# Simencassiman/P2PMicrogrid

Measured on AMD Instinct MI355X. Metric: agent-steps/sec (whole node, rollout+Q-update) at 1/2/4/8 MI355X; % HBM roofline, higher is better.
Workload: dtype f32 simulation, f64 Q-table

## Files before the change

p2pmicrogrid_amd/csrc/p2pmg_fast.hip:

```cpp
#include "p2pmg_fastmath.h"

namespace p2pmg {
namespace {

template <typename QT>
__device__ __forceinline__ Row4<QT> fake_row(const QT* p) {
  const uint32_t x = (uint32_t)(reinterpret_cast<uintptr_t>(p) >> 5);
  return Row4<QT>{{(QT)(x & 3), (QT)((x >> 2) & 3), (QT)((x >> 4) & 3), (QT)0}};
}

template <int N, int D, int G>
__device__ __forceinline__ void gather_even(float ev, float (&col)[N], int i) {
  if constexpr (D < G) {
    const float got = shfl_xor_c<D>(ev);
    const int src = i ^ D;
#pragma unroll
    for (int k = 0; k < N; ++k) col[k] = (k == src) ? got : col[k];
    gather_even<N, D + 1, G>(ev, col, i);
  }
}

#ifndef P2PMG_BAT_SPEC
#define P2PMG_BAT_SPEC 1
#endif
// ... 53 lines not shown
    bk = BatK{p.bat_min, p.bat_max, p.bat_sqrt_eff, recip64_u(p.bat_sqrt_eff), kR900};
    rcap = recip64(bcap > 0.0 ? bcap : 1.0);
  }
  const int ip_zero = idx_plain(div_n<N>(0.0f) / mi, np);
  QT* const q_dummy = reinterpret_cast<QT*>(p.dummy) + lane * kQPad;
  constexpr bool narrow = NARROW;
  const size_t rec_bytes = narrow ? sizeof(float2) : sizeof(FastRec);
  char* const rec_dummy = reinterpret_cast<char*>(reinterpret_cast<FastRec*>(p.dummy) + kWave + lane);
  const bool rec_on = p.record != 0 && active;
  const size_t rec_step = rec_on ? A * rec_bytes : 0;

  auto temp_bin = [&](float t_in) {
    const float x = t_in - k.setpoint;
    return clamp_bin_f(((x + 1.0f) / 2.0f) * km2_T + 1.0f, km1_T);
  };
  auto p2p_bin = [&](float x) { return clamp_bin_f(((x + 1.0f) / 2.0f) * kp, km1_p); };

  const float* envb = p.env + (size_t)s_env * kEnvStride;
  const size_t env_step = (size_t)p.n_env * kEnvStride;
  const uint2* preb = pre + a;
  const uint32_t* ipc_a = p.pre_ipc + a;
  const int t1 = T > 1 ? 1 : 0, t2 = 2 % T;
  const int n_chain = p.chain > 1 ? p.chain : 1;
  bool st_on = active;
  size_t rec_adv = rec_step;
  bool wrap_l = false;
  bool wrap_it = false;
  QT* snap = nullptr;
  if constexpr (PIPE) {
    __shared__ QT snap_lds[2 * 32 * 32];
    snap = snap_lds;
  }
  const uint32_t* codes_a;
  char* rec_ptr;
  uint32_t TA, env_st, env_end, o3, eo3;
  EnvV eS[3];
  uint2 pS[3];
  uint32_t cS[3];
  uint32_t cw, strip, a0, aN;
  int iT;
  Row4<QT> row0, rowN;
  uint32_t iS[3] = {0u, 0u, 0u};
  Row4<QT> cand[3];
  Patch<QT> pat{0xFFFFFFFFu, 0, (QT)0};
  float ep_sum = 0.0f;
  float t0_in = tin, t0_m = tm;
  auto code_of = [&](uint32_t w) { return TRAIN ? w : 0xFFFFFFFFu; };
  auto strip_of = [&](uint32_t base, int it_) { return __umul24(base + __umul24((uint32_t)it_, (uint32_t)nbv), (uint32_t)np); };
  auto row0_addr = [&](uint32_t st, uint32_t nr, uint32_t c) -> uint32_t {
    const bool need = ((c & 0xFF) == 255) || (TRAIN && R1 == 1);
    return need ? st + (uint32_t)ip_zero : nr;
  };
#if P2PMG_TRACE
  uint64_t trW = 0, trC = 0, trR = 0, trLast = 0, trA0 = 0, trWC = 0, trA1 = 0, trMid = 0, trCal = 0;
#define P2PMG_STAMP(v) asm volatile("s_memtime %0\n s_waitcnt lgkmcnt(0)" : "=s"(v)::"memory")
#endif
  auto begin_episode = [&](int ep) __attribute__((always_inline)) {
    if constexpr (PIPE) {
      if (ep >= 1 && st_on) {
        tin = t0_in;
        tm = t0_m;
      }
    }
    codes_a = p.codes + (size_t)(PIPE && ep < 0 ? 0 : ep) * p.codes_stride + a;
    if constexpr (PIPE) {
      rec_ptr = rec_on && st_on ? reinterpret_cast<char*>(recs) + (size_t)a * rec_bytes : rec_dummy;
      rec_adv = st_on ? rec_step : 0;
    } else {
      rec_ptr = rec_on ? reinterpret_cast<char*>(recs) + (size_t)a * rec_bytes : rec_dummy;
    }
    TA = (uint32_t)T * (uint32_t)A, env_st = (uint32_t)env_step, env_end = env_st * (uint32_t)T;
    o3 = (uint32_t)(3 % T) * (uint32_t)A, eo3 = (uint32_t)(3 % T) * env_st;

    eS[0] = load_envv(envb), eS[1] = load_envv(envb + (size_t)t1 * env_step), eS[2] = load_envv(envb + (size_t)t2 * env_step);
    pS[0] = preb[0], pS[1] = preb[(size_t)t1 * A], pS[2] = preb[(size_t)t2 * A];
    cS[0] = codes_a[0], cS[1] = codes_a[(size_t)t1 * A], cS[2] = codes_a[(size_t)t2 * A];
    cw = code_of(cS[0]);
    iT = temp_bin(tin);
    strip = strip_of(pS[0].y & 0xFFFFu, iT);
    const uint32_t nrow = strip_of(pS[0].y >> 16, iT) + (uint32_t)ip_zero;
    a0 = row0_addr(strip, nrow, cw);
    aN = TRAIN ? nrow : a0;
    row0 = gat(a0);
    rowN = gat(aN);
    if constexpr (CAND) {
      iS[0] = ipc_a[0];
      iS[1] = ipc_a[(size_t)t1 * A];
      iS[2] = ipc_a[(size_t)t2 * A];
#pragma unroll
      for (int b = 0; b < 3; ++b) cand[b] = gat((strip + ((iS[0] >> (8 * b)) & 0xFFu)));
    }
    pat = Patch<QT>{0xFFFFFFFFu, 0, (QT)0};
    ep_sum = 0.0f;
    if constexpr (!PIPE) {
      t0_in = tin, t0_m = tm;
      if (p.reset_t0 && active)
        t0_draw(p.seed_lo, p.seed_hi, p.episode + ep + 1, p.agent_offset + (uint32_t)a, k.setpoint, p.reset_sigma, t0_in,
                t0_m);
    } else {
      constexpr int kSnap = 10;
      const uint32_t key0 = pS[0].y & 0xFFFFu;
      const int nTi = p.nT;
      Row4<QT> sr[kSnap];
      auto snap_load = [&](int it0) {
#pragma unroll
        for (int j = 0; j < kSnap; ++j) sr[j] = gat(strip_of(key0, it0 + j < nTi ? it0 + j : nTi - 1) + (uint32_t)ip_zero);
      };
      auto snap_store = [&](int it0) {
#pragma unroll
        for (int j = 0; j < kSnap; ++j)
          if (it0 + j < nTi) snap[(grp * 32 + it0 + j) * 32 + hl] = max3(sr[j]);
      };
      snap_load(0);
      if (active)
        t0_draw(p.seed_lo, p.seed_hi, p.episode + (ep + 2 < n_chain ? ep + 2 : n_chain), p.agent_offset + (uint32_t)a,
                k.setpoint, p.reset_sigma, t0_in, t0_m);
      snap_store(0);
      for (int it0 = kSnap; it0 < nTi; it0 += kSnap) {
        snap_load(it0);
        snap_store(it0);
      }
    }
  };
  auto end_episode = [&](int ep) __attribute__((always_inline)) {
    if (active) {
      if (p.reset_t0) {
        tin = t0_in;
        tm = t0_m;
      }
      if (i == 0) {
        if (p.chain_rewards) p.chain_rewards[(size_t)ep * p.S + s] = ep_sum;
        if (ep == n_chain - 1) p.ep_reward[s] = ep_sum;
      }
    }
  };

  auto step = [&](auto par) __attribute__((always_inline)) {
    constexpr int P = decltype(par)::value, P1 = (P + 1) % 3;
    const EnvV ev = eS[P];
    const EnvRow e0{0.0f, ev.x, ev.y, ev.z, ev.w};
    const uint2 p0 = pS[P], p1 = pS[P1];
    const uint32_t c1 = cS[P1], ipc0 = iS[P], ipc1 = iS[P1];
    const float balw = __uint_as_float(p0.x);
    float row[N];
    float col[N];
#pragma unroll
    for (int j = 0; j < N; ++j) { row[j] = 0.0f; col[j] = 0.0f; }
    float tinA[3];
    uint32_t iTA[3], stA[3], nrA[3];
    {
      const float ain = k.inv_ri * (tm - tin) + k.inv_rvent * (e0.t_out - tin);
#pragma unroll
      for (int x = 0; x < 3; ++x) {
// ... 38 lines not shown
    float tin1 = tin, tm1 = tm;
    int iT1 = 0;
    uint32_t strip1 = 0, cw1 = 0, a0n = 0, aNn = 0;
    Row4<QT> row0n, rowNn, candn[3];
    Sel3M mnext{};
    auto issue_next = [&](int act_final) {
      const Sel3M m = sel3_masks(act_final);
      mnext = m;
      strip1 = __float_as_uint(sel3(m, __uint_as_float(stA[0]), __uint_as_float(stA[1]), __uint_as_float(stA[2])));
      const uint32_t nrow1 =
          __float_as_uint(sel3(m, __uint_as_float(nrA[0]), __uint_as_float(nrA[1]), __uint_as_float(nrA[2])));
      cw1 = code_of(c1);
      a0n = row0_addr(strip1, nrow1, cw1);
      aNn = TRAIN ? nrow1 : a0n;
#if P2PMG_ABLATE == 8 || P2PMG_ABLATE == 10
      row0n = fake_row(q + a0n * kQPad);
      rowNn = fake_row(q + aNn * kQPad);
#else
      {
        Row4<QT> r0{};
        if (((cw1 & 0xFF) == 255) || (TRAIN && R1 == 1)) r0 = gat(a0n);
        row0n = r0;
      }
#endif
      if constexpr (CAND) {
#pragma unroll
        for (int b = 0; b < 3; ++b) candn[b] = gat((strip1 + ((ipc1 >> (8 * b)) & 0xFFu)));
      }
#if !(P2PMG_ABLATE == 8 || P2PMG_ABLATE == 10)
      rowNn = gat(aNn);
#endif
    };
    auto refill_words = [&]() {
      cS[P] = codes_a[o3];
      if constexpr (CAND) iS[P] = ipc_a[o3];
    };
    auto settle_next = [&]() {
      const Sel3M& m = mnext;
      iT1 = (int)__float_as_uint(sel3(m, __uint_as_float(iTA[0]), __uint_as_float(iTA[1]), __uint_as_float(iTA[2])));
      tin1 = sel3(m, tinA[0], tinA[1], tinA[2]);
      const float d_m = k.inv_cm * (((k.inv_ri * (tin - tm) + k.inv_re * (e0.t_out - tm)) + k.solar) +
                                    sel3(m, hm[0], hm[1], hm[2]));
      tm1 = tm + (d_m * k.spm) * k.slot;
    };
    if constexpr (R1 == 1) {
      issue_next(act);
      refill_words();
      settle_next();
    }
    float out0 = balw + hp;
    if constexpr (BAT != 0) {
      if (bcap > 0.0) out0 = bat_rule(out0, soc_r);
    }
    const float ev0 = div_n_r<N>(out0 * 1.0f, rn);
#pragma unroll
    for (int j = 0; j < N; ++j) row[j] = ev0;
#pragma unroll
    for (int r = 1; r < R1; ++r) {
      if (r == 1) {
        gather_even<N, 1, G>(ev0, col, i);
      } else {
        exchange<N>(row, col, i, sl, nullptr);
      }
      code = (int)((cw >> (8 * r)) & 0xFF);
      if (CAND && r == 1) {
        const int b = __float_as_int(shfl_xor_c<1>(__int_as_float(act)));
#if P2PMG_TRACE
// ... 159 lines not shown
      rp[0] = make_float4(rw, cost, g, pp);
      rp[1] = make_float4(tin, __uint_as_float(acts), __uint_as_float(bins), __uint_as_float(ips));
    }
    rec_ptr += PIPE ? rec_adv : rec_step;
    asm volatile("" ::: "memory");
    eS[P] = load_envv(envb + eo3);
    pS[P] = preb[o3];
    const float m = group_sum<N>(rw, lane, i, sl, nullptr);
    ep_sum = ep_sum + div_n_r<N>(m, rn);

    tin = tin1;
    tm = tm1;
    iT = iT1;
    o3 += (uint32_t)A;
    o3 = o3 == TA ? 0u : o3;
    eo3 += env_st;
    eo3 = eo3 == env_end ? 0u : eo3;
    strip = strip1;
    cw = cw1;
    a0 = a0n;
    aN = aNn;
    row0 = row0n;
    rowN = rowNn;
    if constexpr (CAND) {
#pragma unroll
      for (int b = 0; b < 3; ++b) cand[b] = candn[b];
    }
  };
  using S0 = std::integral_constant<int, 0>;
  using S1 = std::integral_constant<int, 1>;
  using S2 = std::integral_constant<int, 2>;
  if constexpr (!PIPE) {
    for (int ep = 0; ep < n_chain; ++ep) {
      begin_episode(ep);
      __builtin_amdgcn_s_waitcnt(0);
      int t = 0;
      for (; t + 3 <= T; t += 3) {
        step(S0{});
        step(S1{});
        step(S2{});
      }
      if (t < T) step(S0{});
      if (t + 1 < T) step(S1{});
#if P2PMG_TRACE
      if (threadIdx.x == 0 && (blockIdx.x == 0 || (int)blockIdx.x == n_cons / 2 || (int)blockIdx.x == n_cons - 1))
        printf("TRACE blk %d/%d T %d: per step wait %.1f round0 %.1f waitcand %.1f round1 %.1f issue %.1f rest %.1f "
               "(one stamp %.1f)\n",
               (int)blockIdx.x, n_cons, T, (double)trW / T, (double)trA0 / T, (double)trWC / T, (double)trA1 / T,
               (double)trC / T, (double)trR / (T - 1), (double)trCal / T);
      trW = trC = trR = trLast = trA0 = trWC = trA1 = trMid = trCal = 0;
#endif
      end_episode(ep);
    }
    if (active) {
      p.t_in[a] = tin;
      p.t_m[a] = tm;
      if constexpr (BAT != 0) p.soc[a] = soc;
    }
  } else {
    const int L = T / 2;
    int ep_l = grp == 0 ? 0 : -1;
    st_on = active && grp == 0;
    begin_episode(ep_l);
    __builtin_amdgcn_s_waitcnt(0);
    for (int ph = 0;; ++ph) {
      if (ph > 0) {
        if (grp == (ph & 1)) {
          if (st_on && i == 0) {
            if (p.chain_rewards) p.chain_rewards[(size_t)ep_l * p.S + s] = ep_sum;
            if (ep_l == n_chain - 1) p.ep_reward[s] = ep_sum;
          }
          if (ph <= n_chain) {
            ep_l = ph;
            st_on = active && ph < n_chain;
            begin_episode(ph < n_chain ? ph : n_chain - 1);
          }
        }
        __builtin_amdgcn_s_waitcnt(0);
        if (ph > n_chain) break;
      }
      wrap_l = st_on && grp != (ph & 1) && ep_l + 1 < n_chain;
      for (int t = 0; t < L; t += 3) {
        wrap_it = t + 3 >= L;
        step(S0{});
        step(S1{});
        step(S2{});
      }
    }
    if (active && grp == ((n_chain - 1) & 1)) {
      p.t_in[a] = t0_in;
      p.t_m[a] = t0_m;
    }
  }
}

template <int N>
constexpr bool kFastPipe = N == 2;

template <int N, typename QT, int R1, int BAT, bool NARROW>
void launch_fast_nw(const EpisodeParams& p, const uint2* pre, FastRec* recs, int blocks, int spw, int prod,
                    const PrepOut& nxt, hipEvent_t ev0, hipEvent_t ev1, hipStream_t st) {
  if constexpr (kFastPipe<N> && BAT == 0) {
    if (p.mode == 0 && p.interleave)
      return hipExtLaunchKernelGGL((episode_fast_kernel<N, QT, R1, true, BAT, NARROW, true>), dim3(blocks + prod),
                                   dim3(kWave), 0, st, ev0, ev1, 0, p, pre, recs, spw, blocks, nxt);
  }
  if (p.mode == 0)
    hipExtLaunchKernelGGL((episode_fast_kernel<N, QT, R1, true, BAT, NARROW>), dim3(blocks + prod), dim3(kWave), 0, st,
                          ev0, ev1, 0, p, pre, recs, spw, blocks, nxt);
  else
    hipExtLaunchKernelGGL((episode_fast_kernel<N, QT, R1, false, BAT, NARROW>), dim3(blocks + prod), dim3(kWave), 0, st,
                          ev0, ev1, 0, p, pre, recs, spw, blocks, nxt);
}
template <int N, typename QT, int R1, int BAT>
void launch_fast_b(const EpisodeParams& p, const uint2* pre, FastRec* recs, int blocks, int spw, int prod,
                   const PrepOut& nxt, hipEvent_t ev0, hipEvent_t ev1, hipStream_t st) {
  if (p.rec_narrow) return launch_fast_nw<N, QT, R1, BAT, true>(p, pre, recs, blocks, spw, prod, nxt, ev0, ev1, st);
  launch_fast_nw<N, QT, R1, BAT, false>(p, pre, recs, blocks, spw, prod, nxt, ev0, ev1, st);
}
template <int N, typename QT, int R1>
void launch_fast_r(const EpisodeParams& p, const uint2* pre, FastRec* recs, int blocks, int spw, int prod,
// ... 73 lines not shown
```

p2pmicrogrid_amd/csrc/p2pmg_fastmath.h:

```cpp
#pragma once
#include "p2pmg_tabular.h"

namespace p2pmg {
namespace {

struct Recip {
  float b, y;
  bool ok;
};
__device__ __forceinline__ bool in_div_range(float x) {
  const float m = fabsf(x);
  return m >= 0x1p-40f && m <= 0x1p40f;
}
__device__ __forceinline__ Recip recip(float b) {
  const float y0 = __builtin_amdgcn_rcpf(b);
  return Recip{b, __builtin_fmaf(__builtin_fmaf(-b, y0, 1.0f), y0, y0), in_div_range(b)};
}
__device__ __forceinline__ float fdiv_core(float a, const Recip& d) {
  const float q0 = a * d.y;
  const float r = __builtin_fmaf(-d.b, q0, a);
  const float q = __builtin_fmaf(r, d.y, q0);
  return __builtin_copysignf(q, q0);
}
__device__ __forceinline__ bool fdiv_ok(float a) {
// ... 26 lines not shown
  const double ang = 6.283185307179586 * u2;
  t_in = (float)((double)setpoint + sigma * (rad * cos(ang)));
  t_m = (float)((double)setpoint + sigma * (rad * sin(ang)));
}
__device__ __forceinline__ void prepass_one(const EpisodeParams& p, const PrepOut& o, size_t k, int ep = 0) {
  const int t = (int)(k / p.A), a = (int)(k % p.A);
  const int tn = t + 1 == p.T ? 0 : t + 1;
  const int se = p.n_env == 1 ? 0 : a / p.N;
  const float mi = p.max_in[a];
  const float2 f = p.prof[k], fn = p.prof[(size_t)tn * p.A + a];
  const float bal = (f.x - f.y) / mi, baln = (fn.x - fn.y) / mi;
  const float time_t = p.env[((size_t)t * p.n_env + se) * kEnvStride];
  const float time_n = p.env[((size_t)tn * p.n_env + se) * kEnvStride];
  const uint32_t tb = (uint32_t)(p.nT * p.nb);
  const uint32_t lo = (uint32_t)idx_time(time_t, p.nt) * tb + (uint32_t)idx_plain(bal, p.nb);
  const uint32_t hi = (uint32_t)idx_time(time_n, p.nt) * tb + (uint32_t)idx_plain(baln, p.nb);
  if (ep == 0) o.pre[k] = make_uint2(__float_as_uint(bal * mi), lo | (hi << 16));
  if (o.ipc && ep == 0) {
    const int i = a % 2, ap = a ^ 1;
    const float2 fp = p.prof[(size_t)t * p.A + ap];
    const float mip = p.max_in[ap];
    const float balw_p = ((fp.x - fp.y) / mip) * mip;
    const float4 lvp = p.hp_lv[ap];
    const float hpl[3] = {lvp.x, lvp.y, lvp.z};
    uint32_t ipc = 0;
    for (int b = 0; b < 3; ++b) {
      const float ev = div_n<2>((balw_p + hpl[b]) * 1.0f);
      float acc = 0.0f;
      for (int j = 0; j < 2; ++j) acc = acc + (-((j == i) ? 0.0f : ev));
      ipc |= (uint32_t)idx_plain(div_n<2>(acc) / mi, p.np) << (8 * b);
    }
    o.ipc[k] = ipc;
  }
  if (o.words) {
    EpisodeParams q = p;
    const bool chain = o.n_ep > 1;
    q.episode = o.episode + ep;
    q.eps = o.eps;
    q.eps_thr = chain ? o.ep_thr[ep] : o.eps_thr;
    q.eps_all = chain ? (int)((o.ep_all >> ep) & 1u) : o.eps_all;
    const int R1 = p.R + 1, W = (R1 + 3) >> 2;
    const uint32_t gid = p.agent_offset + (uint32_t)a;
    const uint64_t codes = philox_codes_of(q, t, gid);
    uint32_t* words = o.words + (size_t)ep * o.words_stride;
    for (int w = 0; w < W; ++w)
      words[((size_t)t * W + w) * p.A + a] =
          w < 2 ? (uint32_t)(codes >> (32 * w))
                : philox_code_word(t, R1, w, (uint32_t)q.episode, gid, q.eps_thr, q.eps_all, p.seed_lo, p.seed_hi);
  }
}

struct Recip64 {
  double d, y;
  bool ok;
};
__device__ __forceinline__ bool in_div_range64(double x) {
  const double m = fabs(x);
  return m >= 0x1p-300 && m <= 0x1p300;
}
__device__ __forceinline__ Recip64 recip64(double d) {
  const double r0 = __builtin_amdgcn_rcp(d);
  const double r1 = __builtin_fma(r0, __builtin_fma(-d, r0, 1.0), r0);
  return Recip64{d, __builtin_fma(r1, __builtin_fma(-d, r1, 1.0), r1), in_div_range64(d)};
}
constexpr Recip64 kR900{900.0, 1.0 / 900.0, true};
__device__ __forceinline__ double fdiv64_ieee(double n, double d) {
// ... 111 lines not shown
```

p2pmicrogrid_amd/csrc/p2pmg_internal.h:

```cpp
#pragma once
#include <hip/hip_runtime.h>
#include <stdint.h>

namespace p2pmg {

constexpr int kEnvStride = 8;
constexpr int kQPad = 4;
constexpr int kWave = 64;
constexpr int kMaxAgents = 64;
constexpr int kMaxRounds1 = 4096;
inline constexpr int general_tile_cap(int n) { return n <= 16 ? 16 : (n <= 32 ? 32 : 64); }
constexpr double kDeltaScale = 1099511627776.0;
constexpr int kDeltaCopies = 8;

struct EpisodeParams {
  int S, N, R, T, A;
  int mode, rng, episode, record;
  int n_env;
  const float* env;
  const float2* prof;
  const uint2* sqp;
  const float* max_in;
  float* t_in;
  float* t_m;
  void* q;
  const uint32_t* codes;
  double eps;
  uint32_t eps_thr;
  int eps_all;
  uint32_t seed_lo, seed_hi;
  uint32_t agent_offset;
  float* rec_reward;
  float* rec_cost;
  float* rec_grid;
  float* rec_p2p;
  float* rec_tin;
  uint8_t* rec_action;
  int32_t* rec_index;
  float* ep_reward;
  int shared_q;
  long long* qdelta;
  int battery;
  double* soc;
  const double* bat_cap;
  double bat_min, bat_max, bat_sqrt_eff;
  int bat_safe;
  const float4* hp_lv;
  const float4* thermal;
  void* dummy;
  uint32_t* pre_ipc;
  void* rec_pack;
  int rec_narrow;
  int reset_t0;
  double reset_sigma;
  int chain;
  int interleave;
  size_t codes_stride;
  float* chain_rewards;
  int nt, nT, nb, np;
  double alpha, gamma;
  float hp_levels[4];
  float setpoint, margin, lower, upper;
  float inv_ci, inv_cm, inv_ri, inv_re, inv_rvent, c_in, c_m, solar, cop, spm, slot;
  float mph, kilo, penw;
};

constexpr int kNetStride = 4672;
constexpr int kOffW1 = 0, kOffB1 = 320, kOffW2 = 384, kOffB2 = 4480, kOffW3 = 4544, kOffB3 = 4608;
constexpr int kDqnParams = 4609;
constexpr int kDqnBatch = 32;
constexpr int kTrans = 10;
constexpr uint32_t kTagSample = 0x5EED0100u;

struct DqnParams {
  EpisodeParams e;
  int t;
  int n_nets;
  float* theta;
  float* target;
  float* adam_m;
  float* adam_v;
  float* grad;
  float* segs;
  int seg_first;
  int n_segs;
  int seg_agents;
  int bps;
// ... 18 lines not shown
  int adam_pending;
  int adam_tpb;
  int fold_spt;
};
hipError_t launch_dqn_act(const DqnParams& p, hipStream_t stream);
hipError_t launch_dqn_sample(const DqnParams& p, hipStream_t stream);
hipError_t launch_dqn_sample_prepass(const DqnParams& p, uint16_t* out, hipStream_t stream);
hipError_t launch_dqn_train(const DqnParams& p, int blocks, bool shared_partials, hipStream_t stream);
int dqn_train_blocks_per_cu();
hipError_t launch_dqn_reduce_adam(const DqnParams& p, int segments, bool adam, hipStream_t stream);
hipError_t launch_dqn_adam_shared(const DqnParams& p, hipStream_t stream);
constexpr int kActAdamSegs = 8;
bool dqn_act_fuses_adam(const DqnParams& p);
hipError_t launch_dqn_forward(const float* theta, int n, const float* x, float* q, hipStream_t stream);

struct RcParams {
  float inv_ci, inv_cm, inv_ri, inv_re, inv_rvent, c_in, c_m, solar, cop, spm, slot;
};

hipError_t launch_episode(const EpisodeParams& p, int q_dtype, int tile, hipStream_t stream);
constexpr int kMaxChain = 64;
struct PrepOut {
  uint2* pre;
  uint32_t* ipc;
  uint32_t* words;
  int episode;
  double eps;
  uint32_t eps_thr;
  int eps_all;
  int n_ep;
  size_t words_stride;
  uint32_t ep_thr[kMaxChain];
  uint64_t ep_all;
};
inline void eps_threshold(double eps, uint32_t& thr, int& all) {
  double c = __builtin_ceil(eps * 4294967296.0);
  if (!(c > 0.0)) c = 0.0;
  all = c >= 4294967296.0 ? 1 : 0;
  thr = all ? 0xFFFFFFFFu : (uint32_t)c;
}
hipError_t launch_step_prepass(const EpisodeParams& p, const PrepOut& o, hipStream_t stream);
constexpr int kChainLagMaxT = 512;
hipError_t launch_chain_lag(int T, int A, const uint2* pre, int* out, hipStream_t stream);
hipError_t launch_episode_fast(const EpisodeParams& p, const uint2* pre, void* recs, int q_dtype, int spw,
                               const PrepOut* next, hipEvent_t ev0, hipEvent_t ev1, hipStream_t stream);
#define P2PMG_DECL_FAST(name)                                                                                     \
  hipError_t name(const EpisodeParams& p, const uint2* pre, void* recs, int q_dtype, int spw, const PrepOut* next, \
                  hipEvent_t ev0, hipEvent_t ev1, hipStream_t stream);
P2PMG_DECL_FAST(launch_fast_n12)
P2PMG_DECL_FAST(launch_fast_n34)
P2PMG_DECL_FAST(launch_fast_n56)
P2PMG_DECL_FAST(launch_fast_n78)
hipError_t launch_general_n1_4(const EpisodeParams& p, int q_dtype, hipStream_t stream);
hipError_t launch_general_n5_8(const EpisodeParams& p, int q_dtype, hipStream_t stream);
hipError_t launch_general_n16(const EpisodeParams& p, int q_dtype, hipStream_t stream);
hipError_t launch_general_tile16(const EpisodeParams& p, int q_dtype, int nc, hipStream_t stream);
hipError_t launch_general_tile32_64(const EpisodeParams& p, int q_dtype, int nc, hipStream_t stream);
hipError_t launch_role_n1_4(const EpisodeParams& p, int q_dtype, hipStream_t stream);
hipError_t launch_role_n5_8(const EpisodeParams& p, int q_dtype, hipStream_t stream);
hipError_t launch_role_n16_tile16(const EpisodeParams& p, int q_dtype, int nc, hipStream_t stream);
hipError_t launch_role_tile32_64(const EpisodeParams& p, int q_dtype, int nc, hipStream_t stream);
hipError_t launch_rule_episode(const EpisodeParams& p, float* hp_on, hipStream_t stream);
hipError_t launch_episode_sq16(const EpisodeParams& p, int q_dtype, hipEvent_t ev0, hipEvent_t ev1, hipStream_t stream);
hipError_t launch_sq16_prep(const EpisodeParams& p, uint2* out, hipStream_t stream);
constexpr size_t kFastRecBytes = 32;
constexpr int kFastBatMaxR1 = 2;
// ... 65 lines not shown
```

p2pmicrogrid_amd/csrc/p2pmg_runtime.cpp:

```cpp
#include "p2pmg.h"

#include <dlfcn.h>
#include <hip/hip_runtime.h>

#include <algorithm>
#include <climits>
#include <cmath>
#include <cstdint>
#include <cstdio>
#include <cstdlib>
#include <cstring>
#include <new>
#include <string>
#include <vector>

#include "p2pmg_internal.h"
#include "p2pmg_plan.h"

using p2pmg::EpisodeParams;
using p2pmg::EpisodePlan;
using p2pmg::Family;
using p2pmg::kEnvStride;
using p2pmg::kQPad;

// ... 65 lines not shown
  int mask = 0;
  int packed_mask = 0;
  int narrow = 0;
  bool timed = false;
  std::string kernel;
};

struct p2pmg_ctx : p2pmg::PlanFacts {
  int device = 0;
  size_t n_states = 0;
  size_t q_elem = 8;
  Stream stream;
  static constexpr int kRing = 4096;
  EventRing ring;
  long long n_timed = 0;
  static constexpr int kCRing = 1024;
  EventRing cring;
  long long n_coll = 0;
  double coll_folded_ms = 0.0;
  long long n_coll_folded = 0;
  int timing_period = 1;
  long long n_launch = 0;
  LastLaunch last;
  DevBuf<float> env;
  DevBuf<float2> prof;
  DevBuf<uint2> sqp;
  long long sqp_version = -1;
  DevBuf<float> max_in, t_in, t_m;
  DevBuf<char> q;
  DevBuf<uint32_t> codes;
  DevBuf<uint2> pre[2];
  DevBuf<uint32_t> pre_ipc[2];
  DevBuf<uint32_t> pcodes[2];
  int pslot = 0;
  bool spec_valid[2] = {false, false};
  int spec_episode[2] = {0, 0};
  std::vector<double> spec_chain[2];
  DevBuf<float> chain_rew;
  int chain_n = 0;
  PinBuf<char> h_small;
  long long spec_version[2] = {-1, -1};
  long long inputs_version = 0;
  long long spec_hits = 0, spec_misses = 0;
  DevBuf<int> d_lag;
  int chain_lag = -1;
  long long lag_version = -1;
  DevBuf<char> dummy;
  DevBuf<char> rec_pack;
  int code_src = 0;
  DevBuf<float> ep_reward;
  DevBuf<float> rec_f32[5];
  DevBuf<uint8_t> rec_action;
  DevBuf<int32_t> rec_index;
  DevBuf<char> rec_stage;
  DevBuf<double> sum_agent, sum_scen;
  DevBuf<float4> hp_lv;
  DevBuf<float4> thermal;
  DevBuf<float> hp_on;
  DevBuf<double> soc, bat_cap;
  bool bat_domain = false;
  bool prof_bounded = false;
  bool hp_bounded = true;
  double bat_min = 0.1, bat_max = 0.9, bat_sqrt_eff = 1.0;
  size_t n_tables = 0;
  DevBuf<long long> qdelta;
  size_t delta_n() const { return n_tables * n_states * kQPad; }
  void* comm = nullptr;
  int rank = 0, nranks = 1;
  p2pmg_exchange_fn xfn = nullptr;
// ... 529 lines not shown
  p.penw = g.penalty_weight;
  return p;
}

static int dqn_run_episode(p2pmg_ctx* c, const p2pmg_episode_args* args);

struct ChainReq {
  int n;
  const double* eps;
  int next_n;
  const double* next_eps;
  float* rewards;
  int reserve;
};

static int run_episode_impl(p2pmg_ctx* c, const p2pmg_episode_args* args, const ChainReq* ch);

int p2pmg_run_episode(p2pmg_ctx* c, const p2pmg_episode_args* args) {
  if (c) c->chain_n = 0;
  return run_episode_impl(c, args, nullptr);
}

static int ensure_rec_pack(p2pmg_ctx* c, const p2pmg_episode_args* args) {
  if (args->record && !c->rec_pack) HIP_TRY(c, c->rec_pack.alloc((size_t)c->T * c->A * p2pmg::kFastRecBytes));
  return P2PMG_OK;
}

static int prepare_fast(p2pmg_ctx* c, const p2pmg_episode_args* args, const ChainReq* ch, const EpisodePlan& plan,
                        EpisodeParams& p, p2pmg::PrepOut* next) {
  const int ps = c->pslot;
  const size_t ta = (size_t)c->T * c->A;
  const size_t wpe = ta * ((c->R + 4) / 4);
  const bool philox = plan.philox == p2pmg::Philox::FastPrepass;
  std::vector<double> cur(ch ? ch->eps : &args->epsilon, ch ? ch->eps + ch->n : &args->epsilon + 1);
  std::vector<double> nxt_eps;
  if (ch) {
    if (ch->next_n > 0) nxt_eps.assign(ch->next_eps, ch->next_eps + ch->next_n);
    else nxt_eps.assign(cur.size(), cur.back());
  } else {
    const bool have_next = (args->flags & P2PMG_FLAG_NEXT_EPSILON) != 0 || args->next_epsilon > 0.0;
    nxt_eps.assign(1, have_next ? args->next_epsilon : args->epsilon);
  }
  const int n_ep = (int)cur.size(), n_next = (int)nxt_eps.size();
  for (int k = 0; k < 2; ++k) {
    if (!c->pre[k]) HIP_TRY(c, c->pre[k].alloc(ta));
    if (plan.want_ipc && !c->pre_ipc[k]) HIP_TRY(c, c->pre_ipc[k].alloc(ta));
    const size_t need = wpe * (size_t)std::max(n_ep, n_next);
    if (philox && c->pcodes[k].cap() < need) {
      c->spec_valid[k] = false;
      HIP_TRY(c, c->pcodes[k].alloc(std::max(need, wpe * (size_t)(ch ? ch->reserve : 1))));
    }
  }
  p.pre_ipc = plan.want_ipc ? c->pre_ipc[ps].get() : nullptr;
  if (philox) p.codes = c->pcodes[ps];
  p.rng = 0;
  p.chain = n_ep;
  p.codes_stride = wpe;
  p.chain_rewards = ch ? ch->rewards : nullptr;
  RC_TRY(ensure_rec_pack(c, args));
  auto prep_out = [&](int slot, int episode, const std::vector<double>& eps) {
    p2pmg::PrepOut o{c->pre[slot], plan.want_ipc ? c->pre_ipc[slot].get() : nullptr,
                     philox ? c->pcodes[slot].get() : nullptr, episode, eps[0], 0u, 0};
    p2pmg::eps_threshold(eps[0], o.eps_thr, o.eps_all);
    o.n_ep = (int)eps.size();
    o.words_stride = wpe;
    o.ep_all = 0;
    for (int k = 0; k < o.n_ep; ++k) {
      int all = 0;
      p2pmg::eps_threshold(eps[k], o.ep_thr[k], all);
      o.ep_all |= (uint64_t)all << k;
    }
    return o;
  };
  const bool hit = c->spec_valid[ps] && c->spec_version[ps] == c->inputs_version &&
                   (!philox || (c->spec_episode[ps] == args->episode && c->spec_chain[ps] == cur));
  if (!hit) HIP_TRY(c, p2pmg::launch_step_prepass(p, prep_out(ps, args->episode, cur), c->stream));
  const int ns = ps ^ 1;
  *next = prep_out(ns, args->episode + n_ep, nxt_eps);
  if (hit) c->spec_hits++;
  else c->spec_misses++;
  c->spec_valid[ns] = plan.speculate;
  c->spec_version[ns] = c->inputs_version;
  c->spec_episode[ns] = philox ? args->episode + n_ep : -1;
  c->spec_chain[ns] = nxt_eps;
  return P2PMG_OK;
}

static int prepare_sq16(p2pmg_ctx* c, const p2pmg_episode_args* args, EpisodeParams& p) {
  RC_TRY(ensure_rec_pack(c, args));
  p.rec_pack = c->rec_pack;
  if (!c->sqp) HIP_TRY(c, c->sqp.alloc((size_t)c->T * c->A));
  if (c->sqp_version != c->inputs_version) {
    HIP_TRY(c, p2pmg::launch_sq16_prep(p, c->sqp, c->stream));
    c->sqp_version = c->inputs_version;
  }
  p.sqp = c->sqp;
  return P2PMG_OK;
}

static int prepare_general(p2pmg_ctx* c, const p2pmg_episode_args* args, const EpisodePlan& plan, EpisodeParams& p) {
  RC_TRY(ensure_records(c, args->record));
  bind_records(c, p);
  if (plan.philox != p2pmg::Philox::CodesPrepass) return P2PMG_OK;
  RC_TRY(ensure_codes(c));
  p.codes = c->codes;
  HIP_TRY(c, p2pmg::launch_philox_codes(p, c->codes, c->stream));
  c->code_src = 2;
  c->have_codes = false;
  p.rng = 0;
  return P2PMG_OK;
}

static int update_chain_lag(p2pmg_ctx* c, const uint2* pre) {
  if (c->lag_version == c->inputs_version) return P2PMG_OK;
  c->chain_lag = -1;
  if (c->T <= p2pmg::kChainLagMaxT) {
    if (!c->d_lag) HIP_TRY(c, c->d_lag.alloc(1));
    HIP_TRY(c, p2pmg::launch_chain_lag(c->T, c->A, pre, c->d_lag, c->stream));
    HIP_TRY(c, hipMemcpyAsync(&c->chain_lag, c->d_lag, sizeof(int), hipMemcpyDeviceToHost, c->stream));
    HIP_TRY(c, hipStreamSynchronize(c->stream));
  }
  c->chain_lag_ok = c->chain_lag >= 0 && c->chain_lag + 4 <= c->T / 2;
  c->lag_version = c->inputs_version;
  return P2PMG_OK;
}

static int run_episode_impl(p2pmg_ctx* c, const p2pmg_episode_args* args, const ChainReq* ch) {
  if (!c || !args) return P2PMG_E_INVALID;
  if (c->dqn) return dqn_run_episode(c, args);
  if (!c->have_env || !c->have_prof || !c->have_params)
    return fail(c, P2PMG_E_STATE, "run_episode: env, profiles and agent params must be set first");
  const bool train = args->mode == P2PMG_MODE_TRAIN;
  if (args->mode != P2PMG_MODE_TRAIN && args->mode != P2PMG_MODE_GREEDY) return fail(c, P2PMG_E_INVALID, "mode");
  if (train && args->rng != P2PMG_RNG_REPLAY && args->rng != P2PMG_RNG_PHILOX) return fail(c, P2PMG_E_INVALID, "rng");
  if (train && args->rng == P2PMG_RNG_REPLAY && !c->have_codes)
    return fail(c, P2PMG_E_STATE, "run_episode: replay mode needs p2pmg_set_replay_codes");
  EpisodePlan plan = p2pmg::plan_episode(*c, *args, ch != nullptr, overrides(), ch ? ch->n : 1);
  if (plan.error) return fail(c, P2PMG_E_INVALID, plan.error);
  const p2pmg_config& g = c->cfg;
  const bool fast = plan.family == Family::Fast, sq16 = plan.family == Family::Sq16, tile = plan.family == Family::Tile;
  const bool ext = plan.packed_records;
  EpisodeParams p = episode_params(c, args);
  const int ps = c->pslot;
  p2pmg::PrepOut next{};
  RC_TRY(fast ? prepare_fast(c, args, ch, plan, p, &next) : sq16 ? prepare_sq16(c, args, p) : prepare_general(c, args, plan, p));
  if (fast && ch && c->lag_version != c->inputs_version) {
    RC_TRY(update_chain_lag(c, c->pre[ps]));
    plan = p2pmg::plan_episode(*c, *args, true, overrides(), ch->n);
  }
  p.interleave = plan.interleave ? 1 : 0;
  p.rec_narrow = plan.rec_narrow;
  const bool reset = (args->flags & P2PMG_FLAG_RESET_T0) != 0;
  p.reset_t0 = (ext && reset) ? 1 : 0;
  p.reset_sigma = args->reset_sigma;
  Timed tm;
  RC_TRY(begin_timed(c, true, !ext, &tm));
  hipError_t e = fast   ? p2pmg::launch_episode_fast(p, c->pre[ps], c->rec_pack, g.q_dtype, plan.spw,
                                                    plan.speculate ? &next : nullptr, tm.e0, tm.e1, c->stream)
                 : sq16 ? p2pmg::launch_episode_sq16(p, g.q_dtype, tm.e0, tm.e1, c->stream)
                        : p2pmg::launch_episode(p, g.q_dtype, tile, c->stream);
  if (e != hipSuccess) return fail(c, P2PMG_E_HIP, std::string("episode launch: ") + hipGetErrorString(e));
  RC_TRY(end_timed(c, tm, !ext));
  if (fast) c->pslot ^= 1;
  if (reset && !ext) {
    const uint32_t off = (uint32_t)(g.scenario_offset * c->N);
    HIP_TRY(c, p2pmg::launch_t0_philox(c->A, c->t_in, c->t_m, p.seed_lo, p.seed_hi, args->episode + 1, off,
                                       c->thermal, args->reset_sigma, c->stream));
  }
  finish_launch(c, tm,
                std::string(fast ? "episode_fast_kernel<" : sq16 ? "episode_sq16_kernel<" : "episode_kernel<") +
                    std::to_string(c->N) + (tile ? ",tile" + std::to_string(p2pmg::general_tile_cap(c->N)) : "") + "," +
                    (g.q_dtype == 0 ? "f64" : "f32") + ",R1=" + std::to_string(c->R + 1) +
                    (ext ? (train ? ",train" : ",greedy") : "") + (g.shared_q ? ",shared" : "") + (c->roles ? ",roles" : "") +
                    (c->battery ? (ext && !p.bat_safe ? ",battery,range-checked>" : ",battery>")
                                : plan.interleave ? ",interleaved>" : ">"),
                args->record, ext ? (args->record & 127) : 0, plan.rec_narrow);
  return P2PMG_OK;
}

int p2pmg_run_episodes(p2pmg_ctx* c, const p2pmg_episode_args* args, int n, const double* epsilons, int next_n,
                       const double* next_epsilons) {
  if (!c || !args || n < 1 || !epsilons || (next_n > 0 && !next_epsilons)) return P2PMG_E_INVALID;
  if (!c->dqn && (!c->have_env || !c->have_prof || !c->have_params))
    return fail(c, P2PMG_E_STATE, "run_episodes: env, profiles and agent params must be set first");
  HIP_TRY(c, c->chain_rew.grow((size_t)std::max(n, p2pmg::kMaxChain) * c->S));
  c->chain_n = 0;
  const bool chain = !c->dqn && p2pmg::plan_episode(*c, *args, false, overrides()).philox == p2pmg::Philox::FastPrepass;
// ... 345 lines not shown
  c->hp_bounded = ok;
  HIP_TRY(c, hipMemcpyAsync(c->hp_lv, lv.data(), lv.size() * sizeof(float4), hipMemcpyHostToDevice, c->stream));
  HIP_TRY(c, hipStreamSynchronize(c->stream));
  return P2PMG_OK;
}

int p2pmg_get_hp_levels(p2pmg_ctx* c, float* levels) {
  if (!c || !levels) return P2PMG_E_INVALID;
  std::vector<float4> lv((size_t)c->A);
  HIP_TRY(c, hipMemcpyAsync(lv.data(), c->hp_lv, lv.size() * sizeof(float4), hipMemcpyDeviceToHost, c->stream));
  HIP_TRY(c, hipStreamSynchronize(c->stream));
  for (size_t a = 0; a < lv.size(); ++a) {
    levels[3 * a] = lv[a].x;
    levels[3 * a + 1] = lv[a].y;
    levels[3 * a + 2] = lv[a].z;
  }
  return P2PMG_OK;
}

int p2pmg_set_thermal(p2pmg_ctx* c, const float* params) {
  if (!c) return P2PMG_E_INVALID;
  const p2pmg_config& g = c->cfg;
  std::vector<float4> th((size_t)c->A, make_float4(g.setpoint, g.lower_bound, g.upper_bound, g.hp_cop));
  if (params) {
    for (size_t a = 0; a < th.size(); ++a) {
      const float* v = params + 4 * a;
      if (!(std::isfinite(v[0]) && std::isfinite(v[1]) && std::isfinite(v[2]) && std::isfinite(v[3])))
        return fail(c, P2PMG_E_INVALID, "set_thermal: non-finite value for agent " + std::to_string(a));
      if (v[1] > v[2])
        return fail(c, P2PMG_E_INVALID, "set_thermal: lower bound above upper bound for agent " + std::to_string(a));
      th[a] = make_float4(v[0], v[1], v[2], v[3]);
    }
  }
  HIP_TRY(c, hipMemcpyAsync(c->thermal, th.data(), th.size() * sizeof(float4), hipMemcpyHostToDevice, c->stream));
  HIP_TRY(c, hipStreamSynchronize(c->stream));
  c->thermal_set = params != nullptr;
  return P2PMG_OK;
}

int p2pmg_get_thermal(p2pmg_ctx* c, float* params) {
  if (!c || !params) return P2PMG_E_INVALID;
  static_assert(sizeof(float4) == 4 * sizeof(float), "thermal rows are 4 packed floats");
  HIP_TRY(c, hipMemcpyAsync(params, c->thermal, (size_t)c->A * sizeof(float4), hipMemcpyDeviceToHost, c->stream));
  HIP_TRY(c, hipStreamSynchronize(c->stream));
  return P2PMG_OK;
}

int p2pmg_set_battery(p2pmg_ctx* c, const double* capacity, double min_soc, double max_soc, double efficiency,
                      const double* soc0) {
  if (!c) return P2PMG_E_INVALID;
  c->inputs_version++;
  if (!capacity) {
    c->battery = false;
    return P2PMG_OK;
  }
  if (!(efficiency > 0.0) || !(min_soc <= max_soc)) return fail(c, P2PMG_E_INVALID, "set_battery: bad parameters");
  const size_t A = (size_t)c->A;
  if (!c->bat_cap) HIP_TRY(c, c->bat_cap.alloc(A));
  HIP_TRY(c, hipMemcpyAsync(c->bat_cap, capacity, A * 8, hipMemcpyHostToDevice, c->stream));
  std::vector<double> s0(A, 0.5);
  HIP_TRY(c, hipMemcpyAsync(c->soc, soc0 ? soc0 : s0.data(), A * 8, hipMemcpyHostToDevice, c->stream));
  HIP_TRY(c, hipStreamSynchronize(c->stream));
  {
    auto in = [](double x, double lo, double hi) { return x >= lo && x <= hi; };
    const double se = std::sqrt(efficiency);
    bool ok = in(min_soc, 0x1p-100, 0x1p10) && in(max_soc, 0x1p-100, 0x1p10) && in(se, 0x1p-10, 0x1p10);
// ... 714 lines not shown
```

Baseline: 14.71 billion.

## Precompute t0 resets in prepass and prefetch next-episode words at phase boundaries

Moves the per-episode Philox t0 draw out of the episode kernel into the speculative step prepass, which writes a float2 table that the kernel reads. In the pipelined path the boundary no longer reloads env/pre/code words; instead the tail of the previous phase prefetches the next episode's codes. The Q snapshot load is restructured into one fully unrolled batch of up to 32 rows so more gathers are in flight at once. This adds a t0 buffer, extra speculation-cache keys and higher register pressure, plus optional phase-timing instrumentation.

```diff
diff --git a/p2pmicrogrid_amd/csrc/p2pmg_fast.hip b/p2pmicrogrid_amd/csrc/p2pmg_fast.hip
--- a/p2pmicrogrid_amd/csrc/p2pmg_fast.hip
+++ b/p2pmicrogrid_amd/csrc/p2pmg_fast.hip
@@ -109,6 +109,8 @@
     snap = snap_lds;
   }
   const uint32_t* codes_a;
+  const uint32_t* codes_nx = nullptr;
+  const uint32_t* codes_r = nullptr;
   char* rec_ptr;
   uint32_t TA, env_st, env_end, o3, eo3;
   EnvV eS[3];
@@ -128,30 +130,45 @@
     const bool need = ((c & 0xFF) == 255) || (TRAIN && R1 == 1);
     return need ? st + (uint32_t)ip_zero : nr;
   };
+#if P2PMG_TRACE || P2PMG_TRACE_PHASE
+#define P2PMG_STAMP(v) asm volatile("s_memtime %0\n s_waitcnt lgkmcnt(0)" : "=s"(v)::"memory")
+#endif
 #if P2PMG_TRACE
   uint64_t trW = 0, trC = 0, trR = 0, trLast = 0, trA0 = 0, trWC = 0, trA1 = 0, trMid = 0, trCal = 0;
-#define P2PMG_STAMP(v) asm volatile("s_memtime %0\n s_waitcnt lgkmcnt(0)" : "=s"(v)::"memory")
-#endif
-  auto begin_episode = [&](int ep) __attribute__((always_inline)) {
+#endif
+#if P2PMG_TRACE_PHASE
+  uint64_t trSteps = 0, trBound = 0, trIssue = 0, trRows = 0, trPh = 0;
+#endif
+  auto begin_episode = [&](int ep, auto fill) __attribute__((always_inline)) {
+    constexpr bool FILL = decltype(fill)::value;
     if constexpr (PIPE) {
       if (ep >= 1 && st_on) {
         tin = t0_in;
         tm = t0_m;
       }
-    }
-    codes_a = p.codes + (size_t)(PIPE && ep < 0 ? 0 : ep) * p.codes_stride + a;
-    if constexpr (PIPE) {
+      codes_a = FILL ? p.codes + (size_t)(ep < 0 ? 0 : ep) * p.codes_stride + a : codes_nx;
+      codes_nx = ep + 2 < n_chain ? p.codes + (size_t)(ep + 2) * p.codes_stride + a : codes_a;
+      codes_r = codes_a;
       rec_ptr = rec_on && st_on ? reinterpret_cast<char*>(recs) + (size_t)a * rec_bytes : rec_dummy;
       rec_adv = st_on ? rec_step : 0;
     } else {
+      codes_a = p.codes + (size_t)ep * p.codes_stride + a;
       rec_ptr = rec_on ? reinterpret_cast<char*>(recs) + (size_t)a * rec_bytes : rec_dummy;
     }
-    TA = (uint32_t)T * (uint32_t)A, env_st = (uint32_t)env_step, env_end = env_st * (uint32_t)T;
-    o3 = (uint32_t)(3 % T) * (uint32_t)A, eo3 = (uint32_t)(3 % T) * env_st;
-
-    eS[0] = load_envv(envb), eS[1] = load_envv(envb + (size_t)t1 * env_step), eS[2] = load_envv(envb + (size_t)t2 * env_step);
-    pS[0] = preb[0], pS[1] = preb[(size_t)t1 * A], pS[2] = preb[(size_t)t2 * A];
-    cS[0] = codes_a[0], cS[1] = codes_a[(size_t)t1 * A], cS[2] = codes_a[(size_t)t2 * A];
+    if constexpr (FILL) {
+      TA = (uint32_t)T * (uint32_t)A, env_st = (uint32_t)env_step, env_end = env_st * (uint32_t)T;
+      const int ts = PIPE && ep < 0 ? T / 2 : 0;
+      const size_t s0 = (size_t)ts, s1 = (size_t)(ts + t1), s2 = (size_t)(ts + t2);
+      o3 = (uint32_t)((ts + 3) % T) * (uint32_t)A, eo3 = (uint32_t)((ts + 3) % T) * env_st;
+      eS[0] = load_envv(envb + s0 * env_step), eS[1] = load_envv(envb + s1 * env_step), eS[2] = load_envv(envb + s2 * env_step);
+      pS[0] = preb[s0 * A], pS[1] = preb[s1 * A], pS[2] = preb[s2 * A];
+      cS[0] = codes_a[s0 * A], cS[1] = codes_a[s1 * A], cS[2] = codes_a[s2 * A];
+      if constexpr (CAND) iS[0] = ipc_a[s0 * A], iS[1] = ipc_a[s1 * A], iS[2] = ipc_a[s2 * A];
+    }
+#if P2PMG_TRACE_PHASE
+    uint64_t tpe0, tpe1, tpe2;
+    P2PMG_STAMP(tpe0);
+#endif
     cw = code_of(cS[0]);
     iT = temp_bin(tin);
     strip = strip_of(pS[0].y & 0xFFFFu, iT);
@@ -161,9 +178,6 @@
     row0 = gat(a0);
     rowN = gat(aN);
     if constexpr (CAND) {
-      iS[0] = ipc_a[0];
-      iS[1] = ipc_a[(size_t)t1 * A];
-      iS[2] = ipc_a[(size_t)t2 * A];
 #pragma unroll
       for (int b = 0; b < 3; ++b) cand[b] = gat((strip + ((iS[0] >> (8 * b)) & 0xFFu)));
     }
@@ -171,31 +185,39 @@
     ep_sum = 0.0f;
     if constexpr (!PIPE) {
       t0_in = tin, t0_m = tm;
-      if (p.reset_t0 && active)
-        t0_draw(p.seed_lo, p.seed_hi, p.episode + ep + 1, p.agent_offset + (uint32_t)a, k.setpoint, p.reset_sigma, t0_in,
-                t0_m);
+      if (p.reset_t0) {
+        const float2 d = p.t0[(size_t)ep * A + a];
+        t0_in = d.x, t0_m = d.y;
+      }
     } else {
-      constexpr int kSnap = 10;
+      constexpr int kSnap = 4, kSnapMax = 32;
       const uint32_t key0 = pS[0].y & 0xFFFFu;
       const int nTi = p.nT;
-      Row4<QT> sr[kSnap];
-      auto snap_load = [&](int it0) {
-#pragma unroll
-        for (int j = 0; j < kSnap; ++j) sr[j] = gat(strip_of(key0, it0 + j < nTi ? it0 + j : nTi - 1) + (uint32_t)ip_zero);
-      };
-      auto snap_store = [&](int it0) {
-#pragma unroll
-        for (int j = 0; j < kSnap; ++j)
-          if (it0 + j < nTi) snap[(grp * 32 + it0 + j) * 32 + hl] = max3(sr[j]);
-      };
-      snap_load(0);
-      if (active)
-        t0_draw(p.seed_lo, p.seed_hi, p.episode + (ep + 2 < n_chain ? ep + 2 : n_chain), p.agent_offset + (uint32_t)a,
-                k.setpoint, p.reset_sigma, t0_in, t0_m);
-      snap_store(0);
-      for (int it0 = kSnap; it0 < nTi; it0 += kSnap) {
-        snap_load(it0);
-        snap_store(it0);
+      Row4<QT> sr[kSnapMax];
+#pragma unroll
+      for (int b0 = 0; b0 < kSnapMax; b0 += kSnap) {
+        if (b0 < nTi) {
+#pragma unroll
+          for (int j = b0; j < b0 + kSnap; ++j) sr[j] = gat(strip_of(key0, j < nTi ? j : nTi - 1) + (uint32_t)ip_zero);
+        }
+      }
+      const float2 d = p.t0[(size_t)(ep + 1 < n_chain ? ep + 1 : n_chain - 1) * A + a];
+      t0_in = d.x, t0_m = d.y;
+#if P2PMG_TRACE_PHASE
+      P2PMG_STAMP(tpe1);
+      asm volatile("" ::"v"(row0.v[0]), "v"(rowN.v[0]), "v"(sr[0].v[0]), "v"(t0_in));
+      if (nTi > 16) asm volatile("" ::"v"(sr[16].v[0]));
+      if (nTi > 28) asm volatile("" ::"v"(sr[28].v[0]));
+      P2PMG_STAMP(tpe2);
+      if (!FILL) trIssue += tpe1 - tpe0, trRows += tpe2 - tpe1;
+#endif
+#pragma unroll
+      for (int b0 = 0; b0 < kSnapMax; b0 += kSnap) {
+        if (b0 < nTi) {
+#pragma unroll
+          for (int j = b0; j < b0 + kSnap; ++j)
+            if (j < nTi) snap[(grp * 32 + j) * 32 + hl] = max3(sr[j]);
+        }
       }
     }
   };
@@ -300,7 +322,7 @@
 #endif
     };
     auto refill_words = [&]() {
-      cS[P] = codes_a[o3];
+      cS[P] = (PIPE ? codes_r : codes_a)[o3];
       if constexpr (CAND) iS[P] = ipc_a[o3];
     };
     auto settle_next = [&]() {
@@ -526,7 +548,7 @@
   using S2 = std::integral_constant<int, 2>;
   if constexpr (!PIPE) {
     for (int ep = 0; ep < n_chain; ++ep) {
-      begin_episode(ep);
+      begin_episode(ep, std::true_type{});
       __builtin_amdgcn_s_waitcnt(0);
       int t = 0;
       for (; t + 3 <= T; t += 3) {
@@ -555,10 +577,15 @@
     const int L = T / 2;
     int ep_l = grp == 0 ? 0 : -1;
     st_on = active && grp == 0;
-    begin_episode(ep_l);
+    begin_episode(ep_l, std::true_type{});
     __builtin_amdgcn_s_waitcnt(0);
     for (int ph = 0;; ++ph) {
       if (ph > 0) {
+#if P2PMG_TRACE_PHASE
+        uint64_t tb0, tb1;
+        P2PMG_STAMP(tb0);
+        trSteps += tb0 - trPh;
+#endif
         if (grp == (ph & 1)) {
           if (st_on && i == 0) {
             if (p.chain_rewards) p.chain_rewards[(size_t)ep_l * p.S + s] = ep_sum;
@@ -567,20 +594,34 @@
           if (ph <= n_chain) {
             ep_l = ph;
             st_on = active && ph < n_chain;
-            begin_episode(ph < n_chain ? ph : n_chain - 1);
+            begin_episode(ph < n_chain ? ph : n_chain - 1, std::false_type{});
           }
         }
         __builtin_amdgcn_s_waitcnt(0);
+#if P2PMG_TRACE_PHASE
+        P2PMG_STAMP(tb1);
+        trBound += tb1 - tb0;
+#endif
         if (ph > n_chain) break;
       }
+#if P2PMG_TRACE_PHASE
+      P2PMG_STAMP(trPh);
+#endif
       wrap_l = st_on && grp != (ph & 1) && ep_l + 1 < n_chain;
       for (int t = 0; t < L; t += 3) {
         wrap_it = t + 3 >= L;
+        if (wrap_it) codes_r = grp != (ph & 1) ? codes_nx : codes_a;
         step(S0{});
         step(S1{});
         step(S2{});
       }
     }
+#if P2PMG_TRACE_PHASE
+    if (threadIdx.x == 0 && (blockIdx.x == 0 || (int)blockIdx.x == n_cons / 2 || (int)blockIdx.x == n_cons - 1))
+      printf("PHASE blk %d/%d T %d chain %d: ticks per phase: steps %.1f boundary %.1f (issue %.1f rows %.1f)\n",
+             (int)blockIdx.x, n_cons, T, n_chain, (double)trSteps / (n_chain + 1), (double)trBound / (n_chain + 1),
+             (double)trIssue / (n_chain + 1), (double)trRows / (n_chain + 1));
+#endif
     if (active && grp == ((n_chain - 1) & 1)) {
       p.t_in[a] = t0_in;
       p.t_m[a] = t0_m;
diff --git a/p2pmicrogrid_amd/csrc/p2pmg_fastmath.h b/p2pmicrogrid_amd/csrc/p2pmg_fastmath.h
--- a/p2pmicrogrid_amd/csrc/p2pmg_fastmath.h
+++ b/p2pmicrogrid_amd/csrc/p2pmg_fastmath.h
@@ -82,6 +82,11 @@
     }
     o.ipc[k] = ipc;
   }
+  if (o.t0 && t == 0) {
+    float2 d;
+    t0_draw(p.seed_lo, p.seed_hi, o.episode + ep + 1, p.agent_offset + (uint32_t)a, p.thermal[a].x, o.sigma, d.x, d.y);
+    o.t0[(size_t)ep * p.A + a] = d;
+  }
   if (o.words) {
     EpisodeParams q = p;
     const bool chain = o.n_ep > 1;
diff --git a/p2pmicrogrid_amd/csrc/p2pmg_internal.h b/p2pmicrogrid_amd/csrc/p2pmg_internal.h
--- a/p2pmicrogrid_amd/csrc/p2pmg_internal.h
+++ b/p2pmicrogrid_amd/csrc/p2pmg_internal.h
@@ -53,6 +53,7 @@
   int rec_narrow;
   int reset_t0;
   double reset_sigma;
+  const float2* t0;
   int chain;
   int interleave;
   size_t codes_stride;
@@ -137,6 +138,8 @@
   size_t words_stride;
   uint32_t ep_thr[kMaxChain];
   uint64_t ep_all;
+  float2* t0;
+  double sigma;
 };
 inline void eps_threshold(double eps, uint32_t& thr, int& all) {
   double c = __builtin_ceil(eps * 4294967296.0);
diff --git a/p2pmicrogrid_amd/csrc/p2pmg_runtime.cpp b/p2pmicrogrid_amd/csrc/p2pmg_runtime.cpp
--- a/p2pmicrogrid_amd/csrc/p2pmg_runtime.cpp
+++ b/p2pmicrogrid_amd/csrc/p2pmg_runtime.cpp
@@ -121,9 +121,12 @@
   DevBuf<uint2> pre[2];
   DevBuf<uint32_t> pre_ipc[2];
   DevBuf<uint32_t> pcodes[2];
+  DevBuf<float2> pt0[2];
   int pslot = 0;
   bool spec_valid[2] = {false, false};
   int spec_episode[2] = {0, 0};
+  bool spec_reset[2] = {false, false};
+  double spec_sigma[2] = {0.0, 0.0};
   std::vector<double> spec_chain[2];
   DevBuf<float> chain_rew;
   int chain_n = 0;
@@ -719,6 +722,7 @@
   const size_t ta = (size_t)c->T * c->A;
   const size_t wpe = ta * ((c->R + 4) / 4);
   const bool philox = plan.philox == p2pmg::Philox::FastPrepass;
+  const bool reset = p.reset_t0 != 0;
   std::vector<double> cur(ch ? ch->eps : &args->epsilon, ch ? ch->eps + ch->n : &args->epsilon + 1);
   std::vector<double> nxt_eps;
   if (ch) {
@@ -737,9 +741,15 @@
       c->spec_valid[k] = false;
       HIP_TRY(c, c->pcodes[k].alloc(std::max(need, wpe * (size_t)(ch ? ch->reserve : 1))));
     }
+    const size_t need_t0 = (size_t)c->A * (size_t)std::max(n_ep, n_next);
+    if (reset && c->pt0[k].cap() < need_t0) {
+      c->spec_valid[k] = false;
+      HIP_TRY(c, c->pt0[k].alloc(std::max(need_t0, (size_t)c->A * (size_t)(ch ? ch->reserve : 1))));
+    }
   }
   p.pre_ipc = plan.want_ipc ? c->pre_ipc[ps].get() : nullptr;
   if (philox) p.codes = c->pcodes[ps];
+  p.t0 = reset ? c->pt0[ps].get() : nullptr;
   p.rng = 0;
   p.chain = n_ep;
   p.codes_stride = wpe;
@@ -757,10 +767,15 @@
       p2pmg::eps_threshold(eps[k], o.ep_thr[k], all);
       o.ep_all |= (uint64_t)all << k;
     }
+    o.t0 = reset ? c->pt0[slot].get() : nullptr;
+    o.sigma = p.reset_sigma;
     return o;
   };
   const bool hit = c->spec_valid[ps] && c->spec_version[ps] == c->inputs_version &&
-                   (!philox || (c->spec_episode[ps] == args->episode && c->spec_chain[ps] == cur));
+                   (!philox || (c->spec_episode[ps] == args->episode && c->spec_chain[ps] == cur)) &&
+                   c->spec_reset[ps] == reset &&
+                   (!reset || (c->spec_episode[ps] == args->episode && c->spec_chain[ps].size() == cur.size() &&
+                               c->spec_sigma[ps] == p.reset_sigma));
   if (!hit) HIP_TRY(c, p2pmg::launch_step_prepass(p, prep_out(ps, args->episode, cur), c->stream));
   const int ns = ps ^ 1;
   *next = prep_out(ns, args->episode + n_ep, nxt_eps);
@@ -768,8 +783,10 @@
   else c->spec_misses++;
   c->spec_valid[ns] = plan.speculate;
   c->spec_version[ns] = c->inputs_version;
-  c->spec_episode[ns] = philox ? args->episode + n_ep : -1;
+  c->spec_episode[ns] = philox || reset ? args->episode + n_ep : -1;
   c->spec_chain[ns] = nxt_eps;
+  c->spec_reset[ns] = reset;
+  c->spec_sigma[ns] = p.reset_sigma;
   return P2PMG_OK;
 }
 
@@ -829,6 +846,9 @@
   const bool ext = plan.packed_records;
   EpisodeParams p = episode_params(c, args);
   const int ps = c->pslot;
+  const bool reset = (args->flags & P2PMG_FLAG_RESET_T0) != 0;
+  p.reset_t0 = (ext && reset) ? 1 : 0;
+  p.reset_sigma = args->reset_sigma;
   p2pmg::PrepOut next{};
   RC_TRY(fast ? prepare_fast(c, args, ch, plan, p, &next) : sq16 ? prepare_sq16(c, args, p) : prepare_general(c, args, plan, p));
   if (fast && ch && c->lag_version != c->inputs_version) {
@@ -837,9 +857,6 @@
   }
   p.interleave = plan.interleave ? 1 : 0;
   p.rec_narrow = plan.rec_narrow;
-  const bool reset = (args->flags & P2PMG_FLAG_RESET_T0) != 0;
-  p.reset_t0 = (ext && reset) ? 1 : 0;
-  p.reset_sigma = args->reset_sigma;
   Timed tm;
   RC_TRY(begin_timed(c, true, !ext, &tm));
   hipError_t e = fast   ? p2pmg::launch_episode_fast(p, c->pre[ps], c->rec_pack, g.q_dtype, plan.spw,
@@ -1251,6 +1268,7 @@
       th[a] = make_float4(v[0], v[1], v[2], v[3]);
     }
   }
+  c->inputs_version++;
   HIP_TRY(c, hipMemcpyAsync(c->thermal, th.data(), th.size() * sizeof(float4), hipMemcpyHostToDevice, c->stream));
   HIP_TRY(c, hipStreamSynchronize(c->stream));
   c->thermal_set = params != nullptr;
```

After: 14.54 billion. 0.988x the previous value.
